# QZ1-boy/FCVSR

Hardware: AMD Instinct MI355X
Metric: SR frames/sec (7-frame window, 4x 180x320->720x1280) + PSNR vs ref (higher is better)
Workload: dtype bf16

## Files before the change

### fcvsr_amd/csrc/fft.hip

```cpp
#include <stdlib.h>
#include <string.h>
#include <mutex>
#include "common.h"

namespace fcvsr {

struct FftPlan {
  int N;
  int nfac;
  int fac[20];
  unsigned magic[20];
};

static bool make_plan(int N, FftPlan* p) {
  p->N = N;
  p->nfac = 0;
  int n = N;
  while (n % 8 == 0) { p->fac[p->nfac++] = 8; n /= 8; }
  while (n % 4 == 0) { p->fac[p->nfac++] = 4; n /= 4; }
  while (n % 2 == 0) { p->fac[p->nfac++] = 2; n /= 2; }
  while (n % 9 == 0) { p->fac[p->nfac++] = 9; n /= 9; }
  for (int f = 3; f <= n; f += 2) {
    while (n % f == 0) {
      if (p->nfac >= 20) return false;
// ... 940 lines not shown
  const dim3 grid(cdiv(n, 2 * L), (B * H + 7) / 8 * 8), block((rmax * L + 63) / 64 * 64);
  const size_t lds = 8ull * ts.N * L + 8ull * ts.N;
#define FCVSR_IROWS2(A_, B_) \
  hipLaunchKernelGGL((irfft_rows2_kernel<A_, B_>), grid, block, lds, st, spec, ps, im_off, re_off, n, H, logL, to_view(*dst), scale, tw, B)
  FCVSR_FFT2_DISPATCH(ts, FCVSR_IROWS2);
#undef FCVSR_IROWS2
  if (log) log->two_stage("irfft_rows2", ts, L);
  return 0;
}

static bool pair_ok(const fcvsr_view* v) {
  const int al = v->dtype == FCVSR_F32 ? 8 : 4;
  return v->sc == 1 && v->sx % 2 == 0 && v->sy % 2 == 0 && v->sb % 2 == 0 && ((uintptr_t)v->ptr % al) == 0;
}

constexpr long long kFftLdsBudget = 64 * 1024;

static int pick_lanes(int N, int n_lanes_needed) {
  int L = 32;
  while (L > 1 && (16ll * N * L + 8ll * N) > kFftLdsBudget) L >>= 1;
  while (L > 1 && L / 2 >= n_lanes_needed) L >>= 1;
  return L;
}

template <class K>
static hipError_t allow_lds(K kernel, size_t bytes) {
  return hipFuncSetAttribute((const void*)kernel, hipFuncAttributeMaxDynamicSharedMemorySize, (int)bytes);
}

}

using namespace fcvsr;

extern "C" int fcvsr_rfft2(const fcvsr_view* src, int B, int H, int W, int n, float* spec, int64_t pix_stride,
                           int im_off, int re_off, void* stream) {
  FCVSR_CHECK_ARG(src && src->ptr && spec, "null pointer");
  FCVSR_CHECK_ARG(src->dtype == FCVSR_F32 || src->dtype == FCVSR_BF16 || src->dtype == FCVSR_F16, "bad src dtype");
  FCVSR_CHECK_ARG(B > 0 && H > 0 && W > 1 && n > 0 && n <= src->c, "bad sizes");
  FftPlan pw, ph;
  FCVSR_CHECK_ARG(make_plan(W, &pw) && make_plan(H, &ph), "length has too many factors");
  const int Wf = W / 2 + 1;
  hipStream_t st = (hipStream_t)stream;
  const bool spec_ok = pix_stride % 4 == 0 && im_off % 4 == 0 && re_off % 4 == 0 && ((uintptr_t)spec % 16) == 0;
  const bool spec_pair = pix_stride % 2 == 0 && im_off % 2 == 0 && re_off % 2 == 0 && ((uintptr_t)spec % 8) == 0;
  const TwoStage* tsw = two_stage(W);
  const TwoStage* tsh = two_stage_cols(H);
  PathLog log;
  if (tsw && n % 2 == 0 && pair_ok(src) && spec_pair) {
    const int rc = launch_rfft_rows2(*tsw, src, n, B, H, spec, (long long)pix_stride, im_off, re_off, st, &log);
    if (rc) return rc;
    FCVSR_LAUNCH_CHECK();
  } else {
    const int L = pick_lanes(W, (n + 1) / 2);
    FCVSR_CHECK_ARG(16ll * W * L + 8ll * W <= 160 * 1024, "row too long for LDS");
    const size_t lds = 16ull * W * L + 8ull * W;
    (void)allow_lds(rfft_rows_kernel, lds);
    dim3 grid(cdiv(n, 2 * L), (B * H + 7) / 8 * 8);
    const int sal = src->dtype == FCVSR_F32 ? 16 : 8;
    const int vec = (L >= 4 && n % (2 * L) == 0 && src->sc == 1 && src->sx % 4 == 0 && src->sy % 4 == 0 && src->sb % 4 == 0 &&
                     ((uintptr_t)src->ptr % sal) == 0 && spec_ok) ? 1 : 0;
    hipLaunchKernelGGL(rfft_rows_kernel, grid, dim3(512), lds, st, to_view(*src), (int)src->dtype, n, H, W, L, spec,
                       (long long)pix_stride, im_off, re_off, pw, vec, B);
    FCVSR_LAUNCH_CHECK();
    log.plan("rfft_rows", L, vec);
  }
  if (tsh) {
    const int rc = launch_cols2(*tsh, spec, spec, (long long)pix_stride, im_off, re_off, n, Wf, B, false, nullptr, st, &log);
    if (rc) return rc;
    FCVSR_LAUNCH_CHECK();
  } else {
    const int L = pick_lanes(H, n);
    FCVSR_CHECK_ARG(16ll * H * L + 8ll * H <= 160 * 1024, "column too long for LDS");
    const size_t lds = 16ull * H * L + 8ull * H;
    (void)allow_lds(fft_cols_kernel, lds);
    dim3 grid(cdiv(n, L), (B * Wf + 7) / 8 * 8);
    const int vec = (L >= 4 && n % L == 0 && spec_ok) ? 1 : 0;
    hipLaunchKernelGGL(fft_cols_kernel, grid, dim3(512), lds, st, (const float*)spec, spec, (long long)pix_stride, im_off,
                       re_off, n, H, Wf, L, 0, (const float*)nullptr, ph, vec, B);
    FCVSR_LAUNCH_CHECK();
    log.plan("fft_cols", L, vec);
  }
  return log.publish();
}

static int irfft_rows(const float* mid, long long pix_stride, int im_off, int re_off, int n, int B, int H, int W, const FftPlan& pw,
                      bool mid_vec, const fcvsr_view* dst, hipStream_t st, PathLog* log) {
  const TwoStage* tsw = two_stage(W);
  const bool mid_pair = pix_stride % 2 == 0 && im_off % 2 == 0 && re_off % 2 == 0 && ((uintptr_t)mid % 8) == 0;
  if (tsw && n % 2 == 0 && pair_ok(dst) && mid_pair) {
    const int rc = launch_irfft_rows2(*tsw, mid, pix_stride, im_off, re_off, n, B, H, dst, 1.0f / ((float)H * (float)W), st, log);
    if (rc) return rc;
    FCVSR_LAUNCH_CHECK();
  } else {
    const int L = pick_lanes(W, (n + 1) / 2);
    FCVSR_CHECK_ARG(16ll * W * L + 8ll * W <= 160 * 1024, "row too long for LDS");
    const size_t lds = 16ull * W * L + 8ull * W;
    (void)allow_lds(irfft_rows_kernel, lds);
    dim3 grid(cdiv(n, 2 * L), (B * H + 7) / 8 * 8);
    const int vec = (L >= 4 && n % (2 * L) == 0 && mid_vec && dst->sc == 1 && dst->sx % 4 == 0 && dst->sy % 4 == 0 &&
                     dst->sb % 4 == 0 && ((uintptr_t)dst->ptr % 16) == 0) ? 1 : 0;
    hipLaunchKernelGGL(irfft_rows_kernel, grid, dim3(512), lds, st, mid, pix_stride, im_off, re_off, n, H, W, L, to_view(*dst),
                       1.0f / ((float)H * (float)W), pw, vec, B);
    FCVSR_LAUNCH_CHECK();
    if (log) log->plan("irfft_rows", L, vec);
  }
  return 0;
}

extern "C" int fcvsr_irfft2(const float* spec, int64_t pix_stride, int im_off, int re_off, int B, int H, int W, int n,
                            const float* mask, float* work, const fcvsr_view* dst, void* stream) {
  FCVSR_CHECK_ARG(spec && dst && dst->ptr, "null pointer");
  FCVSR_CHECK_ARG(dst->dtype == FCVSR_F32, "f32 only");
  FCVSR_CHECK_ARG(B > 0 && H > 0 && W > 1 && n > 0 && n <= dst->c, "bad sizes");
  FftPlan pw, ph;
  FCVSR_CHECK_ARG(make_plan(W, &pw) && make_plan(H, &ph), "length has too many factors");
  const int Wf = W / 2 + 1;
  hipStream_t st = (hipStream_t)stream;
  float* mid = work ? work : const_cast<float*>(spec);
  const bool spec_ok = pix_stride % 4 == 0 && im_off % 4 == 0 && re_off % 4 == 0 && ((uintptr_t)spec % 16) == 0;
  const TwoStage* tsh = two_stage_cols(H);
  PathLog log;
  if (tsh) {
    const int rc = launch_cols2(*tsh, spec, mid, (long long)pix_stride, im_off, re_off, n, Wf, B, true, mask, st, &log);
    if (rc) return rc;
    FCVSR_LAUNCH_CHECK();
  } else {
    const int L = pick_lanes(H, n);
    FCVSR_CHECK_ARG(16ll * H * L + 8ll * H <= 160 * 1024, "column too long for LDS");
    const size_t lds = 16ull * H * L + 8ull * H;
    (void)allow_lds(fft_cols_kernel, lds);
    dim3 grid(cdiv(n, L), (B * Wf + 7) / 8 * 8);
    const int vec = (L >= 4 && n % L == 0 && spec_ok && ((uintptr_t)mid % 16) == 0) ? 1 : 0;
    hipLaunchKernelGGL(fft_cols_kernel, grid, dim3(512), lds, st, spec, mid, (long long)pix_stride, im_off, re_off, n, H,
                       Wf, L, 1, mask, ph, vec, B);
    FCVSR_LAUNCH_CHECK();
    log.plan("fft_cols", L, vec);
  }
  const int rc = irfft_rows(mid, (long long)pix_stride, im_off, re_off, n, B, H, W, pw, spec_ok && ((uintptr_t)mid % 16) == 0, dst, st, &log);
  return rc ? rc : log.publish();
}

extern "C" int fcvsr_irfft2_bands(const float* spec, int64_t pix_stride, int im_off, int re_off, int B, int H, int W, int n,
                                  const float* masks, int n_bands, float* work, const fcvsr_view* dst, void* stream) {
  FCVSR_CHECK_ARG(spec && masks && work && dst && n_bands >= 1 && n_bands <= 16, "null argument / 1..16 bands");
  FCVSR_CHECK_ARG(B > 0 && H > 0 && W > 1 && n > 0, "bad sizes");
  const int Wf = W / 2 + 1;
  const long long band = (long long)B * H * Wf * pix_stride;
  hipStream_t st = (hipStream_t)stream;
  const TwoStage* tsh = two_stage_bands(H);
  if (!tsh) {
    for (int m = 0; m < n_bands; ++m) {
      const int rc = fcvsr_irfft2(spec, pix_stride, im_off, re_off, B, H, W, n, masks + (long long)m * H * Wf, work, &dst[m], stream);
      if (rc) return rc;
    }
    return 0;
  }
  for (int m = 0; m < n_bands; ++m)
    FCVSR_CHECK_ARG(dst[m].ptr && dst[m].dtype == FCVSR_F32 && n <= dst[m].c, "dst: f32 views with >= n channels");
  PathLog log;
  {
    const int rc = launch_cols2_bands(*tsh, spec, work, band, (long long)pix_stride, im_off, re_off, n, Wf, B, masks, n_bands, st, &log);
    if (rc) return rc;
    FCVSR_LAUNCH_CHECK();
  }
  FftPlan pw;
  FCVSR_CHECK_ARG(make_plan(W, &pw), "length has too many factors");
  for (int m = 0; m < n_bands; ++m) {
    const float* mid = work + (long long)m * band;
    const bool mid_vec = pix_stride % 4 == 0 && im_off % 4 == 0 && re_off % 4 == 0 && ((uintptr_t)mid % 16) == 0;
    const int rc = irfft_rows(mid, (long long)pix_stride, im_off, re_off, n, B, H, W, pw, mid_vec, &dst[m], st, m == 0 ? &log : nullptr);
    if (rc) return rc;
  }
  return log.publish();
}

extern "C" const char* fcvsr_last_fft_path(void) { return g_fft_path; }
```

### fcvsr_amd/engine.py

```python
from __future__ import annotations

import ctypes as C
import math
import weakref
from collections import OrderedDict
from typing import Dict, List, Optional, Tuple

import numpy as np
import torch

from . import hip
from .hip import ACT_LEAKY, ACT_NONE, ACT_PRELU, ACT_RELU, check, lib, ptr, stream_ptr, view


_MASKS: Dict[Tuple[int, int, int], torch.Tensor] = {}


def band_masks_half(Q: int, H: int, W: int) -> torch.Tensor:
    key = (Q, H, W)
    if key not in _MASKS:
        n = 1024
        step = math.sqrt((n / 2) ** 2 + (n / 2) ** 2) / Q
        d2 = (np.arange(-(n // 2), n - n // 2, 1) ** 2).astype(np.float64)
        r2 = np.power(np.sqrt(d2[:, None] + d2[None, :]), 2)
# ... 187 lines not shown
    def _new(dev, *shape, dtype=torch.float32):
        return torch.empty(*shape, device=dev, dtype=dtype)

    def _channel_sum(self, t):
        B, H, W, Cc = t.shape
        nblk = (H * W + 255) // 256
        out = self._new(t.device, B, Cc)
        scratch = self._new(t.device, B * nblk * Cc)
        v = view(t)
        check(lib().fcvsr_channel_sum(C.byref(v), B, H, W, out.data_ptr(), scratch.data_ptr(), scratch.numel(),
                                      stream_ptr()), "fcvsr_channel_sum")
        return out

    def _ca_gate(self, sums, inv_hw, prefix, Bn, c):
        par = self._par
        w1, w2 = par[prefix + ".conv_du.0.weight"], par[prefix + ".conv_du.2.weight"]
        gate = self._new(sums.device, Bn, c)
        check(lib().fcvsr_ca_gate(sums.data_ptr(), inv_hw, w1.data_ptr(), w2.data_ptr(), Bn, c, w1.shape[0],
                                  gate.data_ptr(), stream_ptr()), "fcvsr_ca_gate")
        return gate

    def _mgaa(self, x1, x2, x3, tag):
        m = self._model()
        n, A = m.n_feats, m.ACNum
        dev = x1.device
        B, H, W, _ = x1.shape
        Wf = W // 2 + 1
        L = lib()
        st = stream_ptr()
        par = self._par

        spec = self._new(dev, 3, B, H, Wf, 2 * n)
        fs = 2 * n
        for i, xi in enumerate((x1, x2, x3)):
            v = view(xi)
            check(L.fcvsr_rfft2(C.byref(v), B, H, W, n, spec[i].data_ptr(), fs, 0, n, st), "fcvsr_rfft2")
        x1f, x2f, x3f = spec[0], spec[1], spec[2]

        fdt = self._adt(freq=True)
        off = self._new(dev, 2 * B, H, Wf, 2 * n, dtype=fdt)
        fused = fdt != torch.float32 and n == 64
        if fused:
            ws = [self._weights(f"MGAA.convfuse.{i}", torch.bfloat16)[0] for i in (0, 2, 4)]
            P2 = C.c_void_p * 2
            check(L.fcvsr_freq_mlp3(P2(x1f.data_ptr(), x3f.data_ptr()), P2(x2f.data_ptr(), x2f.data_ptr()), 2, fs,
                                    B * H * Wf, ws[0].data_ptr(), ws[1].data_ptr(), ws[2].data_ptr(),
                                    P2(off[:B].data_ptr(), off[B:].data_ptr()), 2 * n, st), "fcvsr_freq_mlp3")
        else:
            t0 = self._new(dev, 2 * B, H, Wf, 2 * n, dtype=fdt)
            t1 = self._new(dev, 2 * B, H, Wf, 2 * n, dtype=fdt)
            dirs = list(enumerate((x1f, x3f)))
            self._convg("MGAA.convfuse.0", [dict(srcs=[xa, x2f], dst=t0[d * B:(d + 1) * B]) for d, xa in dirs],
                        act=ACT_RELU, freq=True)
            self._convg("MGAA.convfuse.2", [dict(srcs=[t0], dst=t1)], act=ACT_RELU, freq=True)
            self._convg("MGAA.convfuse.4", [dict(srcs=[t1[d * B:(d + 1) * B]], dst=off[d * B:(d + 1) * B], res=[xa, x2f])
                                            for d, xa in dirs], res_scale=[1.0, -1.0], freq=True)
        sim = self._new(dev, B, H, Wf, 4)
        off4 = self._new(dev, 2 * B, H, Wf, 4)
        if fused:
            check(L.fcvsr_freq_head(x2f.data_ptr(), hip.F32, fs, B * H * Wf,
                                    self._weights("MGAA.convcrt.0", torch.bfloat16)[0].data_ptr(), None,
                                    self._weights("MGAA.convcrt.2", torch.bfloat16)[0].data_ptr(), sim.data_ptr(), st),
                  "fcvsr_freq_head(convcrt)")
        else:
            s0 = self._new(dev, B, H, Wf, n, dtype=fdt)
            self._conv("MGAA.convcrt.0", [x2f], s0, act=ACT_RELU, freq=True)
            self._conv("MGAA.convcrt.2", [s0], sim, freq=True)

        if fdt == torch.float32:
# ... 129 lines not shown
                        check(L.fcvsr_warp(C.byref(cur_v), C.byref(o_v), B, H, W, C.byref(s_v), st), "fcvsr_warp")
                        check(L.fcvsr_sac_v(C.byref(s_v), C.byref(k_v), B, H, W, C.byref(v_v), st), "fcvsr_sac_v")
                        check(L.fcvsr_sac_h(C.byref(v_v), C.byref(k_v), C.byref(fv), 0.1, B, H, W, C.byref(d_v), st),
                              "fcvsr_sac_h")
                    cur = dst
        out = self._new(dev, B, H, W, n, dtype=fdt_act)
        self._conv("MGAA.conv3", [al], out, res=[x2])
        if self.taps is not None:
            self._tap(f"mgaa{tag}.off_f", off4[:B])
            self._tap(f"mgaa{tag}.off_b", off4[B:])
            self._tap(f"mgaa{tag}.sim", sim)
            o = offsets.permute(0, 3, 1, 2).reshape(B, 2, A, 2, H, W)
            self.taps[f"mgaa{tag}.offsets_f"] = o[:, 0].contiguous().clone()
            self.taps[f"mgaa{tag}.offsets_b"] = o[:, 1].contiguous().clone()
            self._tap(f"mgaa{tag}.al_f", al[..., :n])
            self._tap(f"mgaa{tag}.al_b", al[..., n:])
            self._tap(f"mgaa{tag}.out", out)
        return out

    def _mffr(self, x, out_dtype=torch.float32):
        m = self._model()
        n, Q = m.n_feats, m.Freq_Inv
        dev = x.device
        B, H, W, _ = x.shape
        Wf = W // 2 + 1
        L = lib()
        st = stream_ptr()
        par = self._par
        masks = self._mask(Q, H, W, dev)
        spec = self._new(dev, B, H, Wf, 2 * n)
        xv = view(x)
        check(L.fcvsr_rfft2(C.byref(xv), B, H, W, n, spec.data_ptr(), 2 * n, 0, n, st), "fcvsr_rfft2")
        bands = self._new(dev, Q, B, H, W, n)
        work = self._new(dev, Q, B, H, Wf, 2 * n)
        bvs = (hip.View * Q)(*[view(bands[q]) for q in range(Q)])
        check(L.fcvsr_irfft2_bands(spec.data_ptr(), 2 * n, 0, n, B, H, W, n, masks.data_ptr(), Q, work.data_ptr(), bvs, st),
              "fcvsr_irfft2_bands")
        freq = [bands[Q - 1 - i] for i in range(Q)]
        s_o = self._new(dev, B, H, W, n)
        nblk = (H * W + 255) // 256
        scratch = self._new(dev, 2 * B * nblk * n)
        sums = self._new(dev, 2, B, n)
        inv_hw = 1.0 / (H * W)
        mean_sum = self._channel_sum(freq[0])
        ab = [(par[f"MFFRblock.DivEnh_block.{i}.a"], par[f"MFFRblock.DivEnh_block.{i}.b"]) for i in range(Q)]
        staged = n % 4 == 0 and 256 % (n // 4) == 0 and all(f.data_ptr() % 16 == 0 for f in freq)
        s_f = self._new(dev, B, H, W, n) if (Q > 4 or not staged) else None
        check(L.fcvsr_divenh(0, 1, freq[0].data_ptr(), (s_f if s_f is not None else s_o).data_ptr(), s_o.data_ptr(),
                             ab[0][0].data_ptr(), ab[0][1].data_ptr(), mean_sum.data_ptr(), inv_hw, None, None, sums.data_ptr(),
                             scratch.data_ptr(), scratch.numel(), B, H, W, n, st), "fcvsr_divenh(reduce)")
        gates = []
        j0 = 0
        for i in range(Q):
            pre = f"MFFRblock.DivEnh_block.{i}"
            a, b = ab[i]
            first = 1 if i == 0 else 0
            g1 = self._ca_gate(sums[0], inv_hw, pre + ".ca", B, n)
            g2 = self._ca_gate(sums[1], inv_hw, pre + ".ca", B, n) if i > 0 else None
            gates.append((g1, g2))
            sums = self._new(dev, 2, B, n)
            nxt = i + 1 < Q
            if staged:
                sa = hip.DivEnhStageArgs()
                if j0 > 0:
                    sa.ck_s_f, sa.ck_s_o = s_f.data_ptr(), s_o.data_ptr()
                for k, j in enumerate(range(j0, i + 1)):
                    sa.f[k], sa.a[k], sa.b[k] = freq[j].data_ptr(), ab[j][0].data_ptr(), ab[j][1].data_ptr()
# ... 413 lines not shown
```

### fcvsr_amd/hip.py

```python
from __future__ import annotations

import ctypes as C
import os
from typing import Optional, Sequence

import numpy as np
import torch

_HERE = os.path.dirname(os.path.abspath(__file__))
LIB_PATH = os.path.join(_HERE, "lib", "libfcvsr_hip.so")

F32, BF16, F16, U8, U16 = 0, 1, 2, 3, 4
ACT_NONE, ACT_RELU, ACT_LEAKY, ACT_PRELU = 0, 1, 2, 3
_DT = {torch.float32: F32, torch.bfloat16: BF16, torch.float16: F16, torch.uint8: U8, torch.uint16: U16}


class View(C.Structure):
    _fields_ = [("ptr", C.c_void_p), ("sb", C.c_int64), ("sy", C.c_int64), ("sx", C.c_int64), ("sc", C.c_int64),
                ("c", C.c_int32), ("dtype", C.c_int32)]


class GcFinishLevel(C.Structure):
    _fields_ = [("partial", C.c_void_p), ("add", C.c_void_p), ("nparts", C.c_int32)]

# ... 55 lines not shown
PROFILE = None
COMPUTE_DTYPE = "f32"
DOMINANT_KERNEL = "conv_direct_kernel"


class HipError(RuntimeError):
    pass


_lib: Optional[C.CDLL] = None

_VP, _I, _I64, _F = C.c_void_p, C.c_int, C.c_int64, C.c_float
_PV = C.POINTER(View)
SIGNATURES = {
    "fcvsr_last_error": [],
    "fcvsr_last_conv_kernel": [],
    "fcvsr_conv2d_wgrad_scratch_elems": [C.c_int] * 7,
    "fcvsr_conv2d_wgrad": [C.c_void_p, C.c_void_p, C.c_int, C.c_int, C.c_int, C.c_int, C.c_int, C.c_int, C.c_int, C.c_void_p, C.c_void_p,
                           C.c_longlong, C.c_int, C.c_void_p],
    "fcvsr_conv2d_wgrad_mfma_eligible": [C.c_int] * 6,
    "fcvsr_conv2d_wgrad_mfma_scratch_elems": [C.c_int] * 7,
    "fcvsr_conv2d_wgrad_mfma": [C.c_void_p, C.c_void_p, C.c_int, C.c_int, C.c_int, C.c_int, C.c_int, C.c_int, C.c_int, C.c_void_p, C.c_void_p,
                                C.c_void_p, C.c_longlong, C.c_int, C.c_int, C.c_void_p],
    "fcvsr_abi_version": [],
    "fcvsr_device_count": [],
    "fcvsr_conv2d": [C.POINTER(ConvDesc), _VP],
    "fcvsr_conv2d_f32mfma": [C.POINTER(ConvDesc), _VP],
    "fcvsr_conv2d_f32mfma_eligible": [C.POINTER(ConvDesc)],
    "fcvsr_conv2d_mfma": [C.POINTER(ConvDesc), _I, _I, _VP],
    "fcvsr_conv2d_mfma_plan": [C.POINTER(ConvDesc), _I, _I, _I, _I, C.c_char_p, _I],
    "fcvsr_rfft2": [_PV, _I, _I, _I, _I, _VP, _I64, _I, _I, _VP],
    "fcvsr_irfft2": [_VP, _I64, _I, _I, _I, _I, _I, _I, _VP, _VP, _PV, _VP],
    "fcvsr_irfft2_bands": [_VP, _I64, _I, _I, _I, _I, _I, _I, _VP, _I, _VP, _PV, _VP],
    "fcvsr_last_fft_path": [],
    "fcvsr_ffl_workspace_elems": [_I, _I, _I],
    "fcvsr_ffl_diff": [_VP, _VP, _I, _I, _I, _I, _I, _VP, _I, _VP],
    "fcvsr_ffl_weight": [_VP, _I64, _I, _I, _I, _I, _I, _F, _F, _VP, C.c_longlong, _VP, _VP],
    "fcvsr_ffl_grad": [_VP, _I, _VP, _F, _I, _I, _I, _I, _I, _VP, _VP, _VP],
    "fcvsr_corr_lookup": [_VP, _VP, _I64, _I, _I, _I, _I, _I, _I, _PV, _VP],
    "fcvsr_channel_sum": [_PV, _I, _I, _I, _VP, _VP, _I64, _VP],
    "fcvsr_ca_gate": [_VP, _F, _VP, _VP, _I, _I, _I, _VP, _VP],
    "fcvsr_convblk_tail": [_VP, _VP, _VP, _I, _I, _I, _I, _VP, _I64, _I, _I, _I, _I, _VP],
    "fcvsr_convblk": [_VP, _VP, _VP, _VP, _I, _VP, _VP, _VP, _I, _I, _I, _I, _VP, _VP, _I64, _VP, _I64, _I, _I, _I, _I, _VP],
    "fcvsr_convblk_heads": [_VP, _I, _VP, _VP, _VP, _VP, _VP, _VP, _I, _I, _I, _VP, _VP, _I64, _VP, _I64, _I, _I, _VP],
    "fcvsr_warp": [_PV, _PV, _I, _I, _I, _PV, _VP],
    "fcvsr_sac_v": [_PV, _PV, _I, _I, _I, _PV, _VP],
    "fcvsr_sac_h": [_PV, _PV, _PV, _F, _I, _I, _I, _PV, _VP],
    "fcvsr_iac_step": [_PV, _PV, _PV, _PV, _F, _I, _I, _I, _PV, _VP],
    "fcvsr_feat_extract": [_PV, _I, _I, _I, _VP, _VP, _I, _VP, _VP, _VP, _I, _VP],
    "fcvsr_freq_head": [_VP, _I, _I64, _I64, _VP, _VP, _VP, _VP, _VP],
    "fcvsr_convcorr_strip": [_VP, _VP, _I, _I, _I, _I, _VP, _VP, _VP, _VP, _VP],
    "fcvsr_freq_mlp3": [_VP, _VP, _I, _I64, _I64, _VP, _VP, _VP, _VP, _I64, _VP],
    "fcvsr_iac_step2": [_PV, _PV, _PV, _PV, _F, _I, _I, _I, _PV, _VP],
    "fcvsr_iac_step2_fused": [_PV, _PV, _PV, _VP, _VP, _PV, _F, _I, _I, _I, _PV, _VP],
    "fcvsr_divenh": [_I, _I, _VP, _VP, _VP, _VP, _VP, _VP, _F, _VP, _VP, _VP, _VP, _I64, _I, _I, _I, _I, _VP],
    "fcvsr_divenh_apply_next": [_I, _VP, _VP, _VP, _VP, _VP, _VP, _F, _VP, _VP, _VP, _VP, _VP, _VP, _VP, _I64, _I, _I, _I, _I, _VP],
    "fcvsr_divenh_stage": [C.POINTER(DivEnhStageArgs), _VP],
    "fcvsr_scale_add": [_VP, _VP, _VP, _I, _VP, _I, _I, _I, _I, _I, _VP],
    "fcvsr_gc_context": [_VP, _VP, _VP, _VP, _I, _I, _I, _I, _VP, _VP, _I64, _VP],
    "fcvsr_gc_finish": [_VP, _I, _VP, _VP, _I, _I, _VP, _VP],
    "fcvsr_gc_apply": [_VP, _VP, _VP, _VP, _I, _F, _I, _I, _I, _I, _VP],
    "fcvsr_xscale": [_VP, _VP, _F, _VP, _VP, _VP, _I, _I, _I, _I, _I, _VP],
    "fcvsr_gc_finish_levels": [C.POINTER(GcFinishLevel), _I, _VP, _VP, _I, _I, _VP],
    "fcvsr_gc_partial_levels": [C.POINTER(GcPartialLevel), _I, _I, _VP, _I, _VP],
    "fcvsr_gc_apply_levels": [C.POINTER(GcApplyLevel), _I, _I, _I, _F, _I, _VP],
    "fcvsr_xscale_levels": [C.POINTER(XscaleLevel), _I, _I, _I, _VP],
# ... 67 lines not shown
    "fcvsr_ensemble_windows_u16": [_VP, _VP, _I, _I, _I, _I, _VP, _I, _I, _I, _VP, _VP, _VP],
    "fcvsr_ensemble_merge": [_VP, _VP, _VP, _VP, _I, _I, _I, _I, _I, _I, _VP, _VP],
    "fcvsr_tile_windows": [_VP, _I, _I, _I, _I, _VP, _I, _I, _VP, _I, _VP, _I, _I, _I, _VP, _VP],
    "fcvsr_tile_windows_u8": [_VP, _VP, _I, _I, _I, _I, _VP, _I, _I, _VP, _I, _VP, _I, _I, _I, _VP, _VP],
    "fcvsr_tile_windows_u16": [_VP, _VP, _I, _I, _I, _I, _VP, _I, _I, _VP, _I, _VP, _I, _I, _I, _VP, _VP],
    "fcvsr_tile_merge": [_VP, _VP, _I, _VP, _I, _I, _I, _VP, _VP, _I, _I, _I, _I, _I, _I, _VP, _VP],
    "fcvsr_tile_pairs_equal": [_VP, _I, _I, _I, _I, _VP, _I, _VP, _I, _VP, _I, _I, _I, _VP, C.c_longlong, _VP, _VP],
    "fcvsr_tile_pairs_equal_u8": [_VP, _I, _I, _I, _I, _VP, _I, _VP, _I, _VP, _I, _I, _I, _VP, C.c_longlong, _VP, _VP],
    "fcvsr_tile_pairs_equal_u16": [_VP, _I, _I, _I, _I, _VP, _I, _VP, _I, _VP, _I, _I, _I, _VP, C.c_longlong, _VP, _VP],
    "fcvsr_tile_windows_sel": [_VP, _I, _I, _I, _I, _VP, _I, _I, _VP, _I, _VP, _I, _I, _I, _VP, _I, _VP, _VP],
    "fcvsr_tile_windows_sel_u8": [_VP, _VP, _I, _I, _I, _I, _VP, _I, _I, _VP, _I, _VP, _I, _I, _I, _VP, _I, _VP, _VP],
    "fcvsr_tile_windows_sel_u16": [_VP, _VP, _I, _I, _I, _I, _VP, _I, _I, _VP, _I, _VP, _I, _I, _I, _VP, _I, _VP, _VP],
    "fcvsr_tile_merge_sel": [_VP, _I, _VP, _VP, _I, _VP, _I, _I, _I, _VP, _VP, _I, _I, _I, _I, _I, _I, _VP, _VP],
    "fcvsr_niqe_scratch_bytes": [_I] * 4,
    "fcvsr_niqe_features": [_VP, C.POINTER(C.c_int64), _I, _I, _I, _I, _I, _I, _I, C.POINTER(C.c_double), _VP, _VP, _VP, C.c_longlong,
                            _VP],
    "fcvsr_brisque_scratch_bytes": [_I] * 3,
    "fcvsr_brisque_features": [_VP, C.POINTER(C.c_int64), _I, _I, _I, _I, _I, _I, C.POINTER(C.c_double), _VP, _VP, C.c_longlong, _VP,
                               _VP],
    "fcvsr_bicubic_downscale": [_VP, _I, C.c_longlong, _I, _I, _I, _VP, _VP],
    "fcvsr_bicubic_upscale": [_VP, _I, C.c_longlong, _I, _I, _I, _VP, _I, _VP],
    "fcvsr_imresize": [_VP, _I, C.c_longlong, _I, _I, _I, _I, _VP, _VP, _I, _VP, _VP, _I, _I, _VP, _I, _VP],
    "fcvsr_frame_pair_sad": [_VP, _I, _I, C.c_longlong, _VP, C.c_longlong, _VP, _VP],
    "fcvsr_frame_line_sums": [_VP, _I, _I, _I, _I, _I, _VP, C.c_longlong, _VP, _VP, _VP],
    "fcvsr_active_compose": [_VP] + [C.c_longlong] * 4 + [_VP, _VP] + [C.c_longlong] * 3 + [_I] * 9 + [_VP, _VP],
    "fcvsr_surface_unpack": [_VP, _I, _I, _I, _I, _VP, _I, _I, _I, _VP, _VP, _VP, _VP],
    "fcvsr_surface_pack": [_VP, _VP, _VP, C.c_longlong, C.c_longlong, C.c_longlong, _I, _I, _I, _I, _VP, _VP],
}
_RESTYPES = {"fcvsr_last_error": C.c_char_p, "fcvsr_last_conv_kernel": C.c_char_p, "fcvsr_last_fft_path": C.c_char_p,
             "fcvsr_conv2d_wgrad_scratch_elems": C.c_longlong,
             "fcvsr_conv2d_wgrad_mfma_scratch_elems": C.c_longlong, "fcvsr_colsum_scratch_elems": C.c_longlong,
             "fcvsr_wgrad_cout1_scratch_elems": C.c_longlong, "fcvsr_conv2d_wgrad_mfma_groups_scratch_elems": C.c_longlong,
             "fcvsr_frame_metrics_scratch_bytes": C.c_longlong, "fcvsr_niqe_scratch_bytes": C.c_longlong,
             "fcvsr_brisque_scratch_bytes": C.c_longlong, "fcvsr_ffl_workspace_elems": C.c_longlong}


def lib() -> C.CDLL:
    global _lib
    if _lib is None:
        if not os.path.exists(LIB_PATH):
            raise HipError(f"{LIB_PATH} not found: run `python -m fcvsr_amd.build` (hipcc, gfx950). "
                           "fcvsr_amd has no CPU fallback.")
        l = C.CDLL(LIB_PATH)
        for name, args in SIGNATURES.items():
            fn = getattr(l, name, None)
            if fn is None:
                continue
            fn.argtypes = args
            fn.restype = _RESTYPES.get(name, C.c_int)
        _lib = l
    return _lib


def check(rc: int, what: str) -> None:
    if rc != 0:
        msg = lib().fcvsr_last_error()
        raise HipError(f"{what} failed (rc={rc}): {msg.decode() if msg else ''}")


def stream_ptr() -> int:
    return torch.cuda.current_stream().cuda_stream


def view(t: torch.Tensor) -> View:
    assert t.dim() == 4, t.shape
    sb, sy, sx, sc = t.stride()
    if t.shape[3] == 1:
# ... 751 lines not shown
```

### include/fcvsr_hip.h

```cpp
#ifndef FCVSR_HIP_H
#define FCVSR_HIP_H

#include <stddef.h>
#include <stdint.h>

#ifdef __cplusplus
extern "C" {
#endif

#define FCVSR_ABI_VERSION 2

enum { FCVSR_E_ARG = -1, FCVSR_E_UNSUPPORTED = -2, FCVSR_E_NOGPU = -3 };
enum { FCVSR_F32 = 0, FCVSR_BF16 = 1, FCVSR_F16 = 2 };
enum { FCVSR_U8 = 3 };
enum { FCVSR_U16 = 4 };
enum { FCVSR_ACT_NONE = 0, FCVSR_ACT_RELU = 1, FCVSR_ACT_LEAKY = 2, FCVSR_ACT_PRELU = 3 };

typedef struct fcvsr_view {
  void*   ptr;
  int64_t sb, sy, sx, sc;
  int32_t c;
  int32_t dtype;
} fcvsr_view;

// ... 62 lines not shown
                              const float* w2, int B, int HW, int C, float* sf_out, float* so_out, float* stats, float* scratch,
                              long long scratch_elems, void* stream);
int fcvsr_divenh_band_backward(const float* f, const float* sf, const float* so, const float* a, const float* b, const float* w1,
                               const float* w2, const float* stats, const float* gsf, const float* gso, int B, int HW, int C, float* gf,
                               float* gsf_out, float* gso_out, float* ga, float* gb, float* dw1, float* dw2, float* scratch,
                               long long scratch_elems, int accumulate, void* stream);
int fcvsr_corr_lookup_bwd(const float* x1f, const float* x2f, int64_t pix_stride, int B, int H, int Wf, int C, int radius, int x_count,
                          const fcvsr_view* g, float* gx1_zeroed, float* gx2_zeroed, void* stream);
int fcvsr_prelu_fwd(const float* x, const float* slope, float* y, long long n, void* stream);
int fcvsr_prelu_bwd(const float* g, const float* x, const float* slope, float* gx, float* gslope, float* scratch, long long n, void* stream);
long long fcvsr_wgrad_cout1_scratch_elems(int B, int H, int C);
int fcvsr_wgrad_cout1(const float* x, const float* gy, int B, int H, int W, int C, float* dw, float* scratch, long long scratch_elems,
                      int accumulate, void* stream);
int fcvsr_iac_bwd_sac(const float* gy, const float* yout, const float* v, const float* s, const fcvsr_view* k1, float slope, int B, int H,
                      int W, int C, float* gfin, int fin_accumulate, float* gv, const fcvsr_view* gk, int k_accumulate, void* stream);
int fcvsr_iac_bwd_warp(const float* gv, const fcvsr_view* k1, const float* prev, const fcvsr_view* off, int B, int H, int W, int C,
                       float* gprev_zeroed, float* goff, void* stream);
int fcvsr_iac_bwd_warp_det_workspace(int B, int H, int W, int C, size_t* bytes);
int fcvsr_iac_bwd_warp_det(const float* gv, const fcvsr_view* k1, const float* prev, const fcvsr_view* off, int B, int H, int W, int C,
                           float* gprev, float* goff, void* workspace, size_t workspace_bytes, void* stream);
long long fcvsr_conv2d_wgrad_mfma_groups_scratch_elems(const int* B, const int* H, const int* W, int n_groups, int cin, int cout, int kh,
                                                       int kw);
int fcvsr_conv2d_wgrad_mfma_groups(const fcvsr_view* xs, const fcvsr_view* gys, const int* B, const int* H, const int* W, int n_groups, int kh,
                                   int kw, int pad, float* dw, float* dbias, float* scratch, long long scratch_elems, int dw_accumulate,
                                   int dbias_accumulate, void* stream);
int fcvsr_up2_adjoint(const float* g, float* out, int B, int H, int W, int C, void* stream);
int fcvsr_pool2_adjoint(const float* g, float* out, int B, int H, int W, int C, void* stream);
int fcvsr_rfft2(const fcvsr_view* src, int B, int H, int W, int n,
                float* spec, int64_t pix_stride, int im_off, int re_off, void* stream);
int fcvsr_irfft2(const float* spec, int64_t pix_stride, int im_off, int re_off, int B, int H, int W, int n,
                 const float* mask, float* work, const fcvsr_view* dst, void* stream);
int fcvsr_irfft2_bands(const float* spec, int64_t pix_stride, int im_off, int re_off, int B, int H, int W, int n,
                       const float* masks, int n_bands, float* work, const fcvsr_view* dst, void* stream);
const char* fcvsr_last_fft_path(void);
long long fcvsr_ffl_workspace_elems(int h, int w, int P);
int fcvsr_ffl_diff(const float* pred, const float* target, int B, int C, int H, int W, int patch_factor, float* d, int d_channels,
                   void* stream);
int fcvsr_ffl_weight(float* spec, int64_t pix_stride, int im_off, int re_off, int h, int w, int P, float alpha, float loss_weight,
                     float* workspace, long long workspace_elems, float* loss, void* stream);
int fcvsr_ffl_grad(const float* r, int r_channels, const float* g_up, float loss_weight, int B, int C, int H, int W, int patch_factor,
                   float* grad_pred, float* grad_target, void* stream);

int fcvsr_feat_extract(const fcvsr_view* x, int B, int H, int W, const void* w, const float* bias, int n_blk,
                       void* const* dst, const int64_t* dst_pix_stride, const int32_t* dst_ch_off, int dst_dtype,
                       void* stream);

int fcvsr_corr_lookup(const float* x1f, const float* x2f, int64_t pix_stride, int B, int H, int Wf, int C, int radius,
                      int x_count, const fcvsr_view* dst, void* stream);
int fcvsr_channel_sum(const fcvsr_view* src, int B, int H, int W, float* out, float* scratch, int64_t scratch_elems,
                      void* stream);
int fcvsr_ca_gate(const float* sum, float inv_hw, const float* w1, const float* w2, int B, int c, int cr,
                  float* gate, void* stream);
int fcvsr_convblk_tail(const float* u, const float* gate, const float* sim, int B, int ndir, int H, int Wf,
                       float* spec, int64_t pix_stride, int re_off, int im_off, int g_stride, int g0, void* stream);
int fcvsr_convblk(const float* x, const float* w1, const float* w2, const float* prelu_slope, int ksize, const float* ca_w1,
                  const float* ca_w2, const float* sim, int B, int ndir, int H, int Wf, float* u_scratch,
                  float* partial_scratch, int64_t partial_elems, float* spec, int64_t pix_stride, int re_off, int im_off,
                  int g_stride, int g0, void* stream);
int fcvsr_convblk_heads(const float* x, int n_heads, const float* const* w1, const float* const* w2,
                        const float* const* prelu_slope, const float* const* ca_w1, const float* const* ca_w2, const float* sim,
                        int B, int H, int Wf, float* u, float* partial, int64_t partial_elems, float* spec, int64_t pix_stride,
                        int re_off, int im_off, void* stream);
int fcvsr_warp(const fcvsr_view* src, const fcvsr_view* off, int B, int H, int W, const fcvsr_view* dst, void* stream);
int fcvsr_sac_v(const fcvsr_view* s, const fcvsr_view* k1, int B, int H, int W, const fcvsr_view* dst, void* stream);
int fcvsr_sac_h(const fcvsr_view* v, const fcvsr_view* k1, const fcvsr_view* feat_in, float slope,
                int B, int H, int W, const fcvsr_view* dst, void* stream);
// ... 261 lines not shown
```

Before: 939.5.

## Block FFT passes over clips to keep spectra cache-resident, batch multi-source rfft2

Adds clip-blocking to the 2D FFT entry points. Each block of clips runs its column and row passes back to back, so the intermediate spectrum can stay in cache within a byte budget instead of streaming the whole batch between passes. Blocking is on by default only for irfft2. A multi-source rfft2 entry now transforms three inputs in one call, interleaved per block. The cost is more, smaller kernel launches, which may underfill the GPU when blocks are small.

```diff
diff --git a/fcvsr_amd/csrc/fft.hip b/fcvsr_amd/csrc/fft.hip
--- a/fcvsr_amd/csrc/fft.hip
+++ b/fcvsr_amd/csrc/fft.hip
@@ -996,22 +996,60 @@
 
 using namespace fcvsr;
 
-extern "C" int fcvsr_rfft2(const fcvsr_view* src, int B, int H, int W, int n, float* spec, int64_t pix_stride,
-                           int im_off, int re_off, void* stream) {
-  FCVSR_CHECK_ARG(src && src->ptr && spec, "null pointer");
-  FCVSR_CHECK_ARG(src->dtype == FCVSR_F32 || src->dtype == FCVSR_BF16 || src->dtype == FCVSR_F16, "bad src dtype");
-  FCVSR_CHECK_ARG(B > 0 && H > 0 && W > 1 && n > 0 && n <= src->c, "bad sizes");
+constexpr long long kFftBlockBudgetBytes = 128ll << 20;
+constexpr bool kBlockRfft2 = false;
+constexpr bool kBlockIrfft2 = true;
+constexpr bool kBlockIrfft2Bands = false;
+
+static long long spectrum_bytes_per_clip(int H, int W, int n) { return 4ll * H * (W / 2 + 1) * 2 * n; }
+
+extern "C" int fcvsr_fft_block_clips(int B, int H, int W, int n, long long passes_bytes_per_clip) {
+  if (B <= 1) return 1;
+  const long long per = passes_bytes_per_clip > 0 ? passes_bytes_per_clip : spectrum_bytes_per_clip(H, W, n);
+  if (per <= 0) return B;
+  const long long kmax = kFftBlockBudgetBytes / per;
+  if (kmax <= 1) return 1;
+  if (kmax >= B) return B;
+  const long long blocks = (B + kmax - 1) / kmax;
+  return (int)((B + blocks - 1) / blocks);
+}
+
+static int resolve_block(int block_clips, bool blocked, int B, long long bytes_per_clip) {
+  if (block_clips > 0) return block_clips < B ? block_clips : B;
+  return blocked ? fcvsr_fft_block_clips(B, 0, 0, 0, bytes_per_clip) : B;
+}
+
+static int bands_block(int B, int H, int W, int n, int n_bands, int block_clips) {
+  return resolve_block(block_clips, kBlockIrfft2Bands, B, (long long)n_bands * spectrum_bytes_per_clip(H, W, n));
+}
+
+extern "C" long long fcvsr_irfft2_bands_work_elems(int B, int H, int W, int n, int64_t pix_stride, int n_bands, int block_clips) {
+  if (B <= 0 || H <= 0 || W <= 1 || n <= 0 || pix_stride <= 0 || n_bands <= 0 || block_clips < 0) return 0;
+  return (long long)n_bands * bands_block(B, H, W, n, n_bands, block_clips) * H * (W / 2 + 1) * (long long)pix_stride;
+}
+
+static fcvsr_view view_at(const fcvsr_view& v, int b0) {
+  fcvsr_view r = v;
+  r.ptr = (char*)v.ptr + (long long)b0 * v.sb * (v.dtype == FCVSR_F32 ? 4 : 2);
+  return r;
+}
+
+struct Fft2Geom {
+  int H, W, n, Wf;
+  long long ps;
+  int im_off, re_off;
   FftPlan pw, ph;
-  FCVSR_CHECK_ARG(make_plan(W, &pw) && make_plan(H, &ph), "length has too many factors");
-  const int Wf = W / 2 + 1;
-  hipStream_t st = (hipStream_t)stream;
-  const bool spec_ok = pix_stride % 4 == 0 && im_off % 4 == 0 && re_off % 4 == 0 && ((uintptr_t)spec % 16) == 0;
-  const bool spec_pair = pix_stride % 2 == 0 && im_off % 2 == 0 && re_off % 2 == 0 && ((uintptr_t)spec % 8) == 0;
-  const TwoStage* tsw = two_stage(W);
-  const TwoStage* tsh = two_stage_cols(H);
-  PathLog log;
+  hipStream_t st;
+  long long clip() const { return (long long)H * Wf * ps; }
+};
+
+static int rfft2_rows(const Fft2Geom& g, const fcvsr_view* src, int B, float* spec, PathLog* log) {
+  const bool spec_ok = g.ps % 4 == 0 && g.im_off % 4 == 0 && g.re_off % 4 == 0 && ((uintptr_t)spec % 16) == 0;
+  const bool spec_pair = g.ps % 2 == 0 && g.im_off % 2 == 0 && g.re_off % 2 == 0 && ((uintptr_t)spec % 8) == 0;
+  const TwoStage* tsw = two_stage(g.W);
+  const int n = g.n, H = g.H, W = g.W;
   if (tsw && n % 2 == 0 && pair_ok(src) && spec_pair) {
-    const int rc = launch_rfft_rows2(*tsw, src, n, B, H, spec, (long long)pix_stride, im_off, re_off, st, &log);
+    const int rc = launch_rfft_rows2(*tsw, src, n, B, H, spec, g.ps, g.im_off, g.re_off, g.st, log);
     if (rc) return rc;
     FCVSR_LAUNCH_CHECK();
   } else {
@@ -1023,13 +1061,20 @@
     const int sal = src->dtype == FCVSR_F32 ? 16 : 8;
     const int vec = (L >= 4 && n % (2 * L) == 0 && src->sc == 1 && src->sx % 4 == 0 && src->sy % 4 == 0 && src->sb % 4 == 0 &&
                      ((uintptr_t)src->ptr % sal) == 0 && spec_ok) ? 1 : 0;
-    hipLaunchKernelGGL(rfft_rows_kernel, grid, dim3(512), lds, st, to_view(*src), (int)src->dtype, n, H, W, L, spec,
-                       (long long)pix_stride, im_off, re_off, pw, vec, B);
+    hipLaunchKernelGGL(rfft_rows_kernel, grid, dim3(512), lds, g.st, to_view(*src), (int)src->dtype, n, H, W, L, spec, g.ps,
+                       g.im_off, g.re_off, g.pw, vec, B);
     FCVSR_LAUNCH_CHECK();
-    log.plan("rfft_rows", L, vec);
-  }
+    if (log) log->plan("rfft_rows", L, vec);
+  }
+  return 0;
+}
+
+static int rfft2_cols(const Fft2Geom& g, int B, float* spec, PathLog* log) {
+  const bool spec_ok = g.ps % 4 == 0 && g.im_off % 4 == 0 && g.re_off % 4 == 0 && ((uintptr_t)spec % 16) == 0;
+  const TwoStage* tsh = two_stage_cols(g.H);
+  const int n = g.n, H = g.H;
   if (tsh) {
-    const int rc = launch_cols2(*tsh, spec, spec, (long long)pix_stride, im_off, re_off, n, Wf, B, false, nullptr, st, &log);
+    const int rc = launch_cols2(*tsh, spec, spec, g.ps, g.im_off, g.re_off, n, g.Wf, B, false, nullptr, g.st, log);
     if (rc) return rc;
     FCVSR_LAUNCH_CHECK();
   } else {
@@ -1037,14 +1082,52 @@
     FCVSR_CHECK_ARG(16ll * H * L + 8ll * H <= 160 * 1024, "column too long for LDS");
     const size_t lds = 16ull * H * L + 8ull * H;
     (void)allow_lds(fft_cols_kernel, lds);
-    dim3 grid(cdiv(n, L), (B * Wf + 7) / 8 * 8);
+    dim3 grid(cdiv(n, L), (B * g.Wf + 7) / 8 * 8);
     const int vec = (L >= 4 && n % L == 0 && spec_ok) ? 1 : 0;
-    hipLaunchKernelGGL(fft_cols_kernel, grid, dim3(512), lds, st, (const float*)spec, spec, (long long)pix_stride, im_off,
-                       re_off, n, H, Wf, L, 0, (const float*)nullptr, ph, vec, B);
+    hipLaunchKernelGGL(fft_cols_kernel, grid, dim3(512), lds, g.st, (const float*)spec, spec, g.ps, g.im_off, g.re_off, n, H,
+                       g.Wf, L, 0, (const float*)nullptr, g.ph, vec, B);
     FCVSR_LAUNCH_CHECK();
-    log.plan("fft_cols", L, vec);
+    if (log) log->plan("fft_cols", L, vec);
+  }
+  return 0;
+}
+
+extern "C" int fcvsr_rfft2_multi(const fcvsr_view* srcs, int n_src, int B, int H, int W, int n, float* const* specs,
+                                 int64_t pix_stride, int im_off, int re_off, int block_clips, void* stream) {
+  FCVSR_CHECK_ARG(srcs && specs && n_src >= 1 && n_src <= 8, "null pointer / 1..8 tensors");
+  FCVSR_CHECK_ARG(B > 0 && H > 0 && W > 1 && n > 0 && block_clips >= 0, "bad sizes");
+  for (int i = 0; i < n_src; ++i) {
+    FCVSR_CHECK_ARG(srcs[i].ptr && specs[i], "null pointer");
+    FCVSR_CHECK_ARG(srcs[i].dtype == FCVSR_F32 || srcs[i].dtype == FCVSR_BF16 || srcs[i].dtype == FCVSR_F16, "bad src dtype");
+    FCVSR_CHECK_ARG(n <= srcs[i].c, "bad sizes");
+  }
+  Fft2Geom g{H, W, n, W / 2 + 1, (long long)pix_stride, im_off, re_off, {}, {}, (hipStream_t)stream};
+  FCVSR_CHECK_ARG(make_plan(W, &g.pw) && make_plan(H, &g.ph), "length has too many factors");
+  const int kb = resolve_block(block_clips, kBlockRfft2, B, spectrum_bytes_per_clip(H, W, n));
+  PathLog log;
+  for (int b0 = 0; b0 < B; b0 += kb) {
+    const int nb = B - b0 < kb ? B - b0 : kb;
+    for (int i = 0; i < n_src; ++i) {
+      PathLog* lg = (b0 == 0 && i == 0) ? &log : nullptr;
+      const fcvsr_view sv = view_at(srcs[i], b0);
+      float* sp = specs[i] + b0 * g.clip();
+      int rc = rfft2_rows(g, &sv, nb, sp, lg);
+      if (!rc) rc = rfft2_cols(g, nb, sp, lg);
+      if (rc) return rc;
+    }
   }
   return log.publish();
+}
+
+extern "C" int fcvsr_rfft2_ex(const fcvsr_view* src, int B, int H, int W, int n, float* spec, int64_t pix_stride,
+                              int im_off, int re_off, int block_clips, void* stream) {
+  FCVSR_CHECK_ARG(src && src->ptr && spec, "null pointer");
+  return fcvsr_rfft2_multi(src, 1, B, H, W, n, &spec, pix_stride, im_off, re_off, block_clips, stream);
+}
+
+extern "C" int fcvsr_rfft2(const fcvsr_view* src, int B, int H, int W, int n, float* spec, int64_t pix_stride,
+                           int im_off, int re_off, void* stream) {
+  return fcvsr_rfft2_ex(src, B, H, W, n, spec, pix_stride, im_off, re_off, 0, stream);
 }
 
 static int irfft_rows(const float* mid, long long pix_stride, int im_off, int re_off, int n, int B, int H, int W, const FftPlan& pw,
@@ -1071,21 +1154,12 @@
   return 0;
 }
 
-extern "C" int fcvsr_irfft2(const float* spec, int64_t pix_stride, int im_off, int re_off, int B, int H, int W, int n,
-                            const float* mask, float* work, const fcvsr_view* dst, void* stream) {
-  FCVSR_CHECK_ARG(spec && dst && dst->ptr, "null pointer");
-  FCVSR_CHECK_ARG(dst->dtype == FCVSR_F32, "f32 only");
-  FCVSR_CHECK_ARG(B > 0 && H > 0 && W > 1 && n > 0 && n <= dst->c, "bad sizes");
-  FftPlan pw, ph;
-  FCVSR_CHECK_ARG(make_plan(W, &pw) && make_plan(H, &ph), "length has too many factors");
-  const int Wf = W / 2 + 1;
-  hipStream_t st = (hipStream_t)stream;
-  float* mid = work ? work : const_cast<float*>(spec);
-  const bool spec_ok = pix_stride % 4 == 0 && im_off % 4 == 0 && re_off % 4 == 0 && ((uintptr_t)spec % 16) == 0;
-  const TwoStage* tsh = two_stage_cols(H);
-  PathLog log;
+static int irfft2_cols(const Fft2Geom& g, const float* spec, float* mid, int B, const float* mask, PathLog* log) {
+  const bool spec_ok = g.ps % 4 == 0 && g.im_off % 4 == 0 && g.re_off % 4 == 0 && ((uintptr_t)spec % 16) == 0;
+  const TwoStage* tsh = two_stage_cols(g.H);
+  const int n = g.n, H = g.H;
   if (tsh) {
-    const int rc = launch_cols2(*tsh, spec, mid, (long long)pix_stride, im_off, re_off, n, Wf, B, true, mask, st, &log);
+    const int rc = launch_cols2(*tsh, spec, mid, g.ps, g.im_off, g.re_off, n, g.Wf, B, true, mask, g.st, log);
     if (rc) return rc;
     FCVSR_LAUNCH_CHECK();
   } else {
@@ -1093,49 +1167,89 @@
     FCVSR_CHECK_ARG(16ll * H * L + 8ll * H <= 160 * 1024, "column too long for LDS");
     const size_t lds = 16ull * H * L + 8ull * H;
     (void)allow_lds(fft_cols_kernel, lds);
-    dim3 grid(cdiv(n, L), (B * Wf + 7) / 8 * 8);
+    dim3 grid(cdiv(n, L), (B * g.Wf + 7) / 8 * 8);
     const int vec = (L >= 4 && n % L == 0 && spec_ok && ((uintptr_t)mid % 16) == 0) ? 1 : 0;
-    hipLaunchKernelGGL(fft_cols_kernel, grid, dim3(512), lds, st, spec, mid, (long long)pix_stride, im_off, re_off, n, H,
-                       Wf, L, 1, mask, ph, vec, B);
+    hipLaunchKernelGGL(fft_cols_kernel, grid, dim3(512), lds, g.st, spec, mid, g.ps, g.im_off, g.re_off, n, H, g.Wf, L, 1, mask,
+                       g.ph, vec, B);
     FCVSR_LAUNCH_CHECK();
-    log.plan("fft_cols", L, vec);
-  }
-  const int rc = irfft_rows(mid, (long long)pix_stride, im_off, re_off, n, B, H, W, pw, spec_ok && ((uintptr_t)mid % 16) == 0, dst, st, &log);
-  return rc ? rc : log.publish();
-}
-
-extern "C" int fcvsr_irfft2_bands(const float* spec, int64_t pix_stride, int im_off, int re_off, int B, int H, int W, int n,
-                                  const float* masks, int n_bands, float* work, const fcvsr_view* dst, void* stream) {
+    if (log) log->plan("fft_cols", L, vec);
+  }
+  return 0;
+}
+
+extern "C" int fcvsr_irfft2_ex(const float* spec, int64_t pix_stride, int im_off, int re_off, int B, int H, int W, int n,
+                               const float* mask, float* work, const fcvsr_view* dst, int block_clips, void* stream) {
+  FCVSR_CHECK_ARG(spec && dst && dst->ptr, "null pointer");
+  FCVSR_CHECK_ARG(dst->dtype == FCVSR_F32, "f32 only");
+  FCVSR_CHECK_ARG(B > 0 && H > 0 && W > 1 && n > 0 && n <= dst->c && block_clips >= 0, "bad sizes");
+  Fft2Geom g{H, W, n, W / 2 + 1, (long long)pix_stride, im_off, re_off, {}, {}, (hipStream_t)stream};
+  FCVSR_CHECK_ARG(make_plan(W, &g.pw) && make_plan(H, &g.ph), "length has too many factors");
+  const int kb = resolve_block(block_clips, kBlockIrfft2, B, spectrum_bytes_per_clip(H, W, n));
+  PathLog log;
+  for (int b0 = 0; b0 < B; b0 += kb) {
+    const int nb = B - b0 < kb ? B - b0 : kb;
+    PathLog* lg = b0 == 0 ? &log : nullptr;
+    const float* sp = spec + b0 * g.clip();
+    float* mid = work ? work : const_cast<float*>(sp);
+    const fcvsr_view dv = view_at(*dst, b0);
+    const bool mid_vec = pix_stride % 4 == 0 && im_off % 4 == 0 && re_off % 4 == 0 && ((uintptr_t)sp % 16) == 0 && ((uintptr_t)mid % 16) == 0;
+    int rc = irfft2_cols(g, sp, mid, nb, mask, lg);
+    if (!rc) rc = irfft_rows(mid, g.ps, im_off, re_off, n, nb, H, W, g.pw, mid_vec, &dv, g.st, lg);
+    if (rc) return rc;
+  }
+  return log.publish();
+}
+
+extern "C" int fcvsr_irfft2(const float* spec, int64_t pix_stride, int im_off, int re_off, int B, int H, int W, int n,
+                            const float* mask, float* work, const fcvsr_view* dst, void* stream) {
+  return fcvsr_irfft2_ex(spec, pix_stride, im_off, re_off, B, H, W, n, mask, work, dst, 0, stream);
+}
+
+extern "C" int fcvsr_irfft2_bands_ex(const float* spec, int64_t pix_stride, int im_off, int re_off, int B, int H, int W, int n,
+                                     const float* masks, int n_bands, float* work, const fcvsr_view* dst, int block_clips,
+                                     void* stream) {
   FCVSR_CHECK_ARG(spec && masks && work && dst && n_bands >= 1 && n_bands <= 16, "null argument / 1..16 bands");
-  FCVSR_CHECK_ARG(B > 0 && H > 0 && W > 1 && n > 0, "bad sizes");
+  FCVSR_CHECK_ARG(B > 0 && H > 0 && W > 1 && n > 0 && block_clips >= 0, "bad sizes");
   const int Wf = W / 2 + 1;
-  const long long band = (long long)B * H * Wf * pix_stride;
+  const int kb = bands_block(B, H, W, n, n_bands, block_clips);
   hipStream_t st = (hipStream_t)stream;
   const TwoStage* tsh = two_stage_bands(H);
   if (!tsh) {
     for (int m = 0; m < n_bands; ++m) {
-      const int rc = fcvsr_irfft2(spec, pix_stride, im_off, re_off, B, H, W, n, masks + (long long)m * H * Wf, work, &dst[m], stream);
+      const int rc = fcvsr_irfft2_ex(spec, pix_stride, im_off, re_off, B, H, W, n, masks + (long long)m * H * Wf, work, &dst[m], kb, stream);
       if (rc) return rc;
     }
     return 0;
   }
   for (int m = 0; m < n_bands; ++m)
     FCVSR_CHECK_ARG(dst[m].ptr && dst[m].dtype == FCVSR_F32 && n <= dst[m].c, "dst: f32 views with >= n channels");
-  PathLog log;
-  {
-    const int rc = launch_cols2_bands(*tsh, spec, work, band, (long long)pix_stride, im_off, re_off, n, Wf, B, masks, n_bands, st, &log);
-    if (rc) return rc;
-    FCVSR_LAUNCH_CHECK();
-  }
   FftPlan pw;
   FCVSR_CHECK_ARG(make_plan(W, &pw), "length has too many factors");
-  for (int m = 0; m < n_bands; ++m) {
-    const float* mid = work + (long long)m * band;
-    const bool mid_vec = pix_stride % 4 == 0 && im_off % 4 == 0 && re_off % 4 == 0 && ((uintptr_t)mid % 16) == 0;
-    const int rc = irfft_rows(mid, (long long)pix_stride, im_off, re_off, n, B, H, W, pw, mid_vec, &dst[m], st, m == 0 ? &log : nullptr);
-    if (rc) return rc;
+  const long long clip = (long long)H * Wf * pix_stride;
+  const long long band = (long long)kb * clip;
+  PathLog log;
+  for (int b0 = 0; b0 < B; b0 += kb) {
+    const int nb = B - b0 < kb ? B - b0 : kb;
+    PathLog* lg = b0 == 0 ? &log : nullptr;
+    {
+      const int rc = launch_cols2_bands(*tsh, spec + b0 * clip, work, band, (long long)pix_stride, im_off, re_off, n, Wf, nb, masks, n_bands, st, lg);
+      if (rc) return rc;
+      FCVSR_LAUNCH_CHECK();
+    }
+    for (int m = 0; m < n_bands; ++m) {
+      const float* mid = work + (long long)m * band;
+      const bool mid_vec = pix_stride % 4 == 0 && im_off % 4 == 0 && re_off % 4 == 0 && ((uintptr_t)mid % 16) == 0;
+      const fcvsr_view dv = view_at(dst[m], b0);
+      const int rc = irfft_rows(mid, (long long)pix_stride, im_off, re_off, n, nb, H, W, pw, mid_vec, &dv, st, m == 0 ? lg : nullptr);
+      if (rc) return rc;
+    }
   }
   return log.publish();
 }
 
+extern "C" int fcvsr_irfft2_bands(const float* spec, int64_t pix_stride, int im_off, int re_off, int B, int H, int W, int n,
+                                  const float* masks, int n_bands, float* work, const fcvsr_view* dst, void* stream) {
+  return fcvsr_irfft2_bands_ex(spec, pix_stride, im_off, re_off, B, H, W, n, masks, n_bands, work, dst, 0, stream);
+}
+
 extern "C" const char* fcvsr_last_fft_path(void) { return g_fft_path; }
diff --git a/fcvsr_amd/engine.py b/fcvsr_amd/engine.py
--- a/fcvsr_amd/engine.py
+++ b/fcvsr_amd/engine.py
@@ -243,9 +243,9 @@
 
         spec = self._new(dev, 3, B, H, Wf, 2 * n)
         fs = 2 * n
-        for i, xi in enumerate((x1, x2, x3)):
-            v = view(xi)
-            check(L.fcvsr_rfft2(C.byref(v), B, H, W, n, spec[i].data_ptr(), fs, 0, n, st), "fcvsr_rfft2")
+        vs = (hip.View * 3)(view(x1), view(x2), view(x3))
+        sps = (C.c_void_p * 3)(*[spec[i].data_ptr() for i in range(3)])
+        check(L.fcvsr_rfft2_multi(vs, 3, B, H, W, n, sps, fs, 0, n, 0, st), "fcvsr_rfft2_multi")
         x1f, x2f, x3f = spec[0], spec[1], spec[2]
 
         fdt = self._adt(freq=True)
@@ -441,7 +441,7 @@
         xv = view(x)
         check(L.fcvsr_rfft2(C.byref(xv), B, H, W, n, spec.data_ptr(), 2 * n, 0, n, st), "fcvsr_rfft2")
         bands = self._new(dev, Q, B, H, W, n)
-        work = self._new(dev, Q, B, H, Wf, 2 * n)
+        work = self._new(dev, L.fcvsr_irfft2_bands_work_elems(B, H, W, n, 2 * n, Q, 0))
         bvs = (hip.View * Q)(*[view(bands[q]) for q in range(Q)])
         check(L.fcvsr_irfft2_bands(spec.data_ptr(), 2 * n, 0, n, B, H, W, n, masks.data_ptr(), Q, work.data_ptr(), bvs, st),
               "fcvsr_irfft2_bands")
diff --git a/fcvsr_amd/hip.py b/fcvsr_amd/hip.py
--- a/fcvsr_amd/hip.py
+++ b/fcvsr_amd/hip.py
@@ -111,6 +111,12 @@
     "fcvsr_rfft2": [_PV, _I, _I, _I, _I, _VP, _I64, _I, _I, _VP],
     "fcvsr_irfft2": [_VP, _I64, _I, _I, _I, _I, _I, _I, _VP, _VP, _PV, _VP],
     "fcvsr_irfft2_bands": [_VP, _I64, _I, _I, _I, _I, _I, _I, _VP, _I, _VP, _PV, _VP],
+    "fcvsr_fft_block_clips": [_I, _I, _I, _I, C.c_longlong],
+    "fcvsr_irfft2_bands_work_elems": [_I, _I, _I, _I, _I64, _I, _I],
+    "fcvsr_rfft2_ex": [_PV, _I, _I, _I, _I, _VP, _I64, _I, _I, _I, _VP],
+    "fcvsr_rfft2_multi": [_PV, _I, _I, _I, _I, _I, C.POINTER(_VP), _I64, _I, _I, _I, _VP],
+    "fcvsr_irfft2_ex": [_VP, _I64, _I, _I, _I, _I, _I, _I, _VP, _VP, _PV, _I, _VP],
+    "fcvsr_irfft2_bands_ex": [_VP, _I64, _I, _I, _I, _I, _I, _I, _VP, _I, _VP, _PV, _I, _VP],
     "fcvsr_last_fft_path": [],
     "fcvsr_ffl_workspace_elems": [_I, _I, _I],
     "fcvsr_ffl_diff": [_VP, _VP, _I, _I, _I, _I, _I, _VP, _I, _VP],
@@ -244,7 +250,8 @@
              "fcvsr_conv2d_wgrad_mfma_scratch_elems": C.c_longlong, "fcvsr_colsum_scratch_elems": C.c_longlong,
              "fcvsr_wgrad_cout1_scratch_elems": C.c_longlong, "fcvsr_conv2d_wgrad_mfma_groups_scratch_elems": C.c_longlong,
              "fcvsr_frame_metrics_scratch_bytes": C.c_longlong, "fcvsr_niqe_scratch_bytes": C.c_longlong,
-             "fcvsr_brisque_scratch_bytes": C.c_longlong, "fcvsr_ffl_workspace_elems": C.c_longlong}
+             "fcvsr_brisque_scratch_bytes": C.c_longlong, "fcvsr_ffl_workspace_elems": C.c_longlong,
+             "fcvsr_irfft2_bands_work_elems": C.c_longlong}
 
 
 def lib() -> C.CDLL:
diff --git a/include/fcvsr_hip.h b/include/fcvsr_hip.h
--- a/include/fcvsr_hip.h
+++ b/include/fcvsr_hip.h
@@ -118,6 +118,16 @@
                  const float* mask, float* work, const fcvsr_view* dst, void* stream);
 int fcvsr_irfft2_bands(const float* spec, int64_t pix_stride, int im_off, int re_off, int B, int H, int W, int n,
                        const float* masks, int n_bands, float* work, const fcvsr_view* dst, void* stream);
+int fcvsr_fft_block_clips(int B, int H, int W, int n, long long passes_bytes_per_clip);
+long long fcvsr_irfft2_bands_work_elems(int B, int H, int W, int n, int64_t pix_stride, int n_bands, int block_clips);
+int fcvsr_rfft2_ex(const fcvsr_view* src, int B, int H, int W, int n,
+                   float* spec, int64_t pix_stride, int im_off, int re_off, int block_clips, void* stream);
+int fcvsr_rfft2_multi(const fcvsr_view* srcs, int n_src, int B, int H, int W, int n,
+                      float* const* specs, int64_t pix_stride, int im_off, int re_off, int block_clips, void* stream);
+int fcvsr_irfft2_ex(const float* spec, int64_t pix_stride, int im_off, int re_off, int B, int H, int W, int n,
+                    const float* mask, float* work, const fcvsr_view* dst, int block_clips, void* stream);
+int fcvsr_irfft2_bands_ex(const float* spec, int64_t pix_stride, int im_off, int re_off, int B, int H, int W, int n,
+                          const float* masks, int n_bands, float* work, const fcvsr_view* dst, int block_clips, void* stream);
 const char* fcvsr_last_fft_path(void);
 long long fcvsr_ffl_workspace_elems(int h, int w, int P);
 int fcvsr_ffl_diff(const float* pred, const float* target, int B, int C, int H, int W, int patch_factor, float* d, int d_channels,
```

After: 936.7. No clear change (-0.3%).
